# WeltXing/PyDyNet

Measured on AMD Instinct MI355X. Metric: training-step samples/sec (6L Llama3, seq=256), higher is better.
Workload: dtype f32

## Files before the change

### pydynet_amd/csrc/common.h

```cpp
#pragma once
#include <hip/hip_runtime.h>
#include <stdint.h>
#include <stdio.h>
#include <string.h>

#define PDN_MAX_DIMS 8

enum {
  PDN_OK = 0,
  PDN_EINVAL = -1,
  PDN_EUNSUPPORTED = -2,
  PDN_EWORKSPACE = -3,
};

void pdn_set_error(const char* fmt, ...);

enum {
  PDN_CNT_ROWRES_CHUNK = 0,
  PDN_CNT_ROWTILE_PLAIN = 1,
  PDN_CNT_ROWTILE_SWIGLU_FWD = 2,
  PDN_CNT_ROWTILE_SWIGLU_BWD = 3,
  PDN_CNT_ROWTILE_ROPE = 4,
  PDN_CNT_ROWTILE_ROWMAX = 5,
  PDN_CNT_ROWRES_CHUNK_EPI = 6,
  PDN_CNT_ATT_P_FWD = 7,
  PDN_CNT_ATT_P_BWD = 8,
  PDN_CNT_ATT_RES_FWD = 9,
  PDN_CNT_ATT_RES_BWD = 10,
  PDN_CNT_ATT_STREAM = 11,
  PDN_CNT_CE_DX_DEFERRED = 12,
  PDN_CNT_CE_DW = 13,
  PDN_CNT_OUTRES = 14,
  PDN_CNT_OUTRES_TN = 15,
  PDN_CNT_LINEAR_RELU_FWD = 16,
  PDN_CNT_LINEAR_DX_MASKED = 17,
  PDN_CNT_CE_SMALL = 18,
  PDN_CNT_TILED_SWIGLU_FWD = 19,
  PDN_CNT_TILED_SWIGLU_BWD = 20,
  PDN_CNT_CONV_QUAD_FWD = 21,
  PDN_CNT_CONV_QUAD_DGRAD = 22,
  PDN_CNT_CONV_QUAD_WGRAD = 23,
  PDN_CNT_PATCH_EMBED_FWD = 24,
  PDN_CNT_PATCH_EMBED_BWD = 25,
  PDN_CNT_L2NORM_FWD = 26,
  PDN_CNT_L2NORM_BWD = 27,
  PDN_CNT_SAMPLE = 28,
  PDN_CNT_DECODE_ROWS = 29,
  PDN_CNT_DECODE_SLOTS = 30,
  PDN_CNT_DECODE_WIDE = 31,
  PDN_CNT_BEAM = 32,
  PDN_CNT_EXTEND = 33,
  PDN_CNT_SPECULATE = 34,
  PDN_CNT_PENALTY = 35,
  PDN_CNT_LOGPROBS = 36,
  PDN_CNT_LMHEAD_SPLIT = 37,
  PDN_CNT_PREFIX = 38,
  PDN_CNT_CE_DX_SPLIT = 39,
  PDN_CNT_CE_DW_SPLIT = 40,
  PDN_CNT_ROWTILE_SPLIT = 41,
  PDN_CNT_OUTRES_TN_SPLIT = 42,
  PDN_CNT_ATT_SEG = 43,
  PDN_CNT_ROW_LOSS = 44,
  PDN_CNT_SMOOTH_LOSS = 45,
  PDN_CNT_OUTRES_SPLIT = 46,
  PDN_CNT_PROJ288_SPLIT = 47,
  PDN_CNT_LOGIT_EDIT = 48,
  PDN_CNT_PERSAMPLE = 49,
  PDN_CNT_SLOTS = 50
};
void pdn_count(int slot);

#define PDN_CHECK_ARG(cond, ...)          \
  do {                                    \
    if (!(cond)) {                        \
      pdn_set_error(__VA_ARGS__);         \
      return PDN_EINVAL;                  \
    }                                     \
  } while (0)

#define PDN_LAUNCH_CHECK()                                            \
  do {                                                                \
    hipError_t _e = hipGetLastError();                                \
    if (_e != hipSuccess) {                                           \
      pdn_set_error("%s:%d launch failed: %s", __FILE__, __LINE__,    \
                    hipGetErrorString(_e));                           \
      return (int)_e;                                                 \
    }                                                                 \
  } while (0)

#define PDN_HIP(call)                                                 \
  do {                                                                \
    hipError_t _e = (call);                                           \
    if (_e != hipSuccess) {                                           \
      pdn_set_error("%s:%d %s: %s", __FILE__, __LINE__, #call,        \
                    hipGetErrorString(_e));                           \
      return (int)_e;                                                 \
    }                                                                 \
  } while (0)

static inline int64_t cdiv64(int64_t a, int64_t b) { return (a + b - 1) / b; }

struct PdnView {
  int ndim;
  int64_t shape[PDN_MAX_DIMS];
  int64_t stride[PDN_MAX_DIMS];
};

__device__ __forceinline__ float wave_sum(float v) {
#pragma unroll
  for (int o = 32; o > 0; o >>= 1) v += __shfl_xor(v, o, 64);
  return v;
}
__device__ __forceinline__ float wave_max(float v) {
#pragma unroll
  for (int o = 32; o > 0; o >>= 1) v = fmaxf(v, __shfl_xor(v, o, 64));
  return v;
}
__device__ __forceinline__ double wave_sum(double v) {
#pragma unroll
  for (int o = 32; o > 0; o >>= 1) v += __shfl_xor(v, o, 64);
  return v;
}

template <typename T>
__device__ __forceinline__ T block_sum(T v, T* smem) {
  v = wave_sum(v);
  const int lane = threadIdx.x & 63, wid = threadIdx.x >> 6, nw = (blockDim.x + 63) >> 6;
  if (nw == 1) return v;
  __syncthreads();
  if (lane == 0) smem[wid] = v;
  __syncthreads();
  T r = (T)0;
  for (int i = 0; i < nw; ++i) r += smem[i];
  return r;
}
__device__ __forceinline__ void lds_barrier() {
  asm volatile("s_waitcnt lgkmcnt(0)" ::: "memory");
  __builtin_amdgcn_s_barrier();
  asm volatile("" ::: "memory");
}
__device__ __forceinline__ float block_sum_lds(float v, float* smem) {
  v = wave_sum(v);
  const int lane = threadIdx.x & 63, wid = threadIdx.x >> 6, nw = (blockDim.x + 63) >> 6;
  if (nw == 1) return v;
  lds_barrier();
  if (lane == 0) smem[wid] = v;
  lds_barrier();
  float r = 0.f;
  for (int i = 0; i < nw; ++i) r += smem[i];
  return r;
}
// ... 23 lines not shown
```

### pydynet_amd/csrc/gemm.hip

```cpp
#include "common.h"
#include <vector>
#include <mutex>
#include <stdlib.h>
#include <stdio.h>
#include <type_traits>

#include "gemm_tiled.h"
#include "gemm_stream.h"
#include "split_tn.h"

struct TileCfg {
  int waves_m, waves_n, wm, wn, bk;
  float eff;
};
static const TileCfg kCfgs[] = {
    {2, 2, 2, 2, 32, 1.00f},
    {4, 1, 1, 3, 32, 0.97f},
    {1, 4, 3, 1, 32, 0.95f},
    {4, 1, 1, 2, 32, 0.85f},
    {1, 4, 2, 1, 32, 0.90f},
    {2, 2, 1, 1, 32, 0.60f},
    {2, 2, 4, 2, 16, 0.85f},
    {2, 2, 2, 4, 16, 1.10f},
    {4, 1, 2, 3, 16, 0.99f},
// ... 57 lines not shown
    PDN_HIP(hipEventSynchronize(r.e1));
    float t = 0.f;
    PDN_HIP(hipEventElapsedTime(&t, r.e0, r.e1));
    tm += t; tf += r.flops; tb += r.bytes; n++;
    (void)hipEventDestroy(r.e0);
    (void)hipEventDestroy(r.e1);
  }
  g_prof.swap(keep);
  if (ms) *ms = tm;
  if (flops) *flops = tf;
  if (bytes) *bytes = tb;
  if (launches) *launches = n;
  return PDN_OK;
}

#define PDN_GEMM_FAMILIES 5
extern "C" int pdn_gemm_prof_collect_families(double* ms5, double* flops5, int64_t* launches5) {
  std::lock_guard<std::mutex> lk(g_prof_mu);
  double ms[PDN_GEMM_FAMILIES] = {0}, fl[PDN_GEMM_FAMILIES] = {0};
  int64_t n[PDN_GEMM_FAMILIES] = {0};
  for (auto& r : g_prof) {
    PDN_HIP(hipEventSynchronize(r.e1));
    float t = 0.f;
    PDN_HIP(hipEventElapsedTime(&t, r.e0, r.e1));
    const int f = r.family == 5 ? 2 : (r.family < 0 || r.family >= PDN_GEMM_FAMILIES ? 0 : r.family);
    ms[f] += t; fl[f] += r.flops; n[f]++;
    (void)hipEventDestroy(r.e0);
    (void)hipEventDestroy(r.e1);
  }
  for (int f = 0; f < PDN_GEMM_FAMILIES; ++f) {
    if (ms5) ms5[f] = ms[f];
    if (flops5) flops5[f] = fl[f];
    if (launches5) launches5[f] = n[f];
  }
  g_prof.clear();
  return PDN_OK;
}

extern "C" int pdn_gemm_prof_collect(double* total_ms, double* total_flops, int64_t* launches) {
  double ms[PDN_GEMM_FAMILIES], fl[PDN_GEMM_FAMILIES];
  int64_t n[PDN_GEMM_FAMILIES];
  int rc = pdn_gemm_prof_collect_families(ms, fl, n);
  if (rc) return rc;
  double tm = 0, tf = 0;
  int64_t tn = 0;
  for (int f = 0; f < PDN_GEMM_FAMILIES; ++f) { tm += ms[f]; tf += fl[f]; tn += n[f]; }
  if (total_ms) *total_ms = tm;
  if (total_flops) *total_flops = tf;
  if (launches) *launches = tn;
  return PDN_OK;
}

int pdn_gemm_outres_tn_plan(int N, int K, int* nw_out, int* k_per_split_out);
int pdn_gemm_outres_tn_launch(const float* X, const float* G, float* C, int N, int K, int64_t ldx, int64_t ldg,
                              int64_t ldc, int64_t slab, int nw, int k_per_split, void* stream);
int pdn_gemm_outres_tn_blocks_launch(const float* X, const float* G, float* C, int N, int K, int64_t ldx, int64_t ldg,
                                     int nb_cols, int nw, int k_per_split, void* stream);
extern "C" int64_t pdn_gemm_outres_workspace_bytes(int M, int K);
extern "C" int pdn_gemm_outres_plan(int M, int K, int* nw, int* kps);
extern "C" int pdn_gemm_outres_ws_f32(const float* A, const float* B, float* C, const float* bias, const float* residual,
                                      int M, int N, int K, int64_t lda, int64_t ldb, int64_t ldc, int b_trans,
                                      void* workspace, int64_t workspace_bytes, void* stream);
extern "C" int pdn_gemm_outres_supported(int M, int N, int K, int64_t lda, int64_t ldb, int64_t ldc, int b_trans);
extern "C" int pdn_gemm_outres_f32(const float* A, const float* B, float* C, const float* bias,
                                   const float* residual, int M, int N, int K, int64_t lda, int64_t ldb,
                                   int64_t ldc, int b_trans, void* stream);
extern "C" int pdn_gemm_rowres_supported(int M, int N, int K, int64_t lda, int64_t ldb, int64_t ldc, int b_trans);
int pdn_rowtile_plain_ok(int M, int N, int b_trans);
extern "C" int pdn_gemm_rowtile_mode(int mode);
int pdn_outres_split_takes(const float* A, const float* B, const float* C, const float* bias, const float* residual, int M,
                           int K, int64_t lda, int64_t ldb, int64_t ldc, int b_trans, int kb, int64_t b_bstride, int splits,
                           void* stream);
int pdn_outres_split_launch(const float* A, const float* B, float* C, const float* bias, const float* residual, int M, int K,
                            int64_t lda, int64_t ldb, int64_t ldc, int b_trans, int kb, int64_t b_bstride, void* stream,
                            int count_slot);
extern "C" int pdn_gemm_rowres_f32(const float* A, const float* B, float* C, const float* bias,
                                   const float* residual, int M, int N, int K, int64_t lda, int64_t ldb,
                                   int64_t ldc, int b_trans, void* stream);
int pdn_gemm_rowres_blocks(const float* A, const float* B, float* C, int M, int N, int K, int64_t lda, int64_t ldb,
                           int64_t ldc, int b_trans, int nblocks, int64_t b_block_stride, void* stream);

extern "C" int64_t pdn_gemm_f32_workspace_bytes(int M, int N, int K, int nbatch) {
  const int64_t base = (int64_t)64 * M * N * (int64_t)nbatch * 4;
  if (!pdn_outres_tn_split_supported(M, N, nbatch, K)) return base;
  return ((base + 255) & ~(int64_t)255) + pdn_outres_tn_split_extra_bytes(K);
}

bool pdn_gemm_narrow_nn_ok(int M, int N, int K, int64_t a_rs, int64_t a_cs, const void* A);
int pdn_gemm_narrow_nn_launch(const float* A, int64_t lda, const float* B, int64_t b_rs, int64_t b_cs, const float* bias,
                              float* C, int64_t ldc, int M, int N, int K, void* stream);
int pdn_gemm_narrow_tn_plan(int Mc, int N, int K, int64_t a_rs, int64_t a_cs, int64_t b_cs, const void* A, int64_t ws_cap_floats,
                            int* kps);
int pdn_gemm_narrow_tn_launch(const float* A, int64_t a_cs, const float* B, int64_t b_rs, float* slabs, int Mc, int N, int K,
                              int kps, int splits, void* stream);

static int gemm_f32_impl(int M, int N, int K, float alpha, const float* A, int64_t a_rs,
                         int64_t a_cs, const float* B, int64_t b_rs, int64_t b_cs, float beta,
                         float* C, int64_t ldc, const float* bias, int nb1, int nb2,
                         int64_t a_bs1, int64_t a_bs2, int64_t b_bs1, int64_t b_bs2,
                         int64_t c_bs1, int64_t c_bs2, const float* residual,
                         float* b_colsum, int colsum_accumulate, void* workspace,
                         int64_t workspace_bytes, void* stream, uint32_t* relu_mask, const uint32_t* grad_mask,
                         float* mask_colsum = nullptr) {
  const bool ext_on = relu_mask || grad_mask;
  PDN_CHECK_ARG(!ext_on || (nb1 == 1 && nb2 == 1 && N % 32 == 0 && !b_colsum),
                "pdn_gemm_f32: the mask epilogues need one batch and N a multiple of 32 (N = %d)", N);
  PDN_CHECK_ARG(M >= 0 && N >= 0 && K >= 0 && nb1 >= 0 && nb2 >= 0, "pdn_gemm_f32: negative extent");
  if (M == 0 || N == 0 || nb1 == 0 || nb2 == 0) return PDN_OK;
  PDN_CHECK_ARG(A && B && C, "pdn_gemm_f32: null operand");
  PDN_CHECK_ARG(ldc >= N, "pdn_gemm_f32: ldc (%lld) < N (%d)", (long long)ldc, N);
  hipStream_t st = (hipStream_t)stream;
  const int nbatch = nb1 * nb2;

  GemmParams p;
  p.A = A; p.B = B; p.C = C; p.bias = bias; p.ws = (float*)workspace;
  p.residual = residual; p.colsum = b_colsum; p.colsum_acc = colsum_accumulate;
  p.relu_mask = relu_mask; p.grad_mask = grad_mask; p.mask_colsum = grad_mask ? mask_colsum : nullptr;
  p.M = M; p.N = N; p.K = K;
  p.a_rs = a_rs; p.a_cs = a_cs; p.b_rs = b_rs; p.b_cs = b_cs; p.ldc = ldc;
  p.nb2 = nb2;
  p.a_bs1 = a_bs1; p.a_bs2 = a_bs2; p.b_bs1 = b_bs1; p.b_bs2 = b_bs2; p.c_bs1 = c_bs1; p.c_bs2 = c_bs2;
  p.alpha = alpha; p.beta = beta;

  const bool a_kin = !(a_rs == 1 && a_cs != 1) || M == 1;
  const bool b_kin = (b_rs == 1 && b_cs != 1) || (b_rs == 1 && N == 1);
  auto al16 = [](const void* q) { return ((uintptr_t)q & 15) == 0; };
  auto m4 = [](int64_t v) { return (v & 3) == 0; };
  bool vec = al16(A) && al16(B) && m4(a_bs1) && m4(a_bs2) && m4(b_bs1) && m4(b_bs2);
  if (a_kin) vec = vec && a_cs == 1 && m4(a_rs) && m4(K);
  else vec = vec && a_rs == 1 && m4(a_cs) && m4(M);
  if (b_kin) vec = vec && b_rs == 1 && m4(b_cs) && m4(K);
  else vec = vec && b_cs == 1 && m4(b_rs) && m4(N);

  if (b_colsum) {
    if (a_kin || b_kin || !vec || nbatch != 1) {
      pdn_set_error("pdn_gemm_f32: b_colsum needs the x^T @ g layout (A m-contiguous, B n-contiguous, aligned, unbatched)");
      return PDN_EUNSUPPORTED;
    }
  }
  if (M <= 4 && !ext_on && nbatch == 1 && !b_colsum && b_cs == 1 && a_cs == 1 && m4(N) && m4(b_rs) && m4(ldc) &&
      al16(B) && al16(C) && (!bias || al16(bias)) && (!residual || al16(residual)) && K > 0 &&
      (K <= 4096 || (int64_t)K <= 4ll * N)) {
    const dim3 g((N + 127) / 128);
    switch (M) {
      case 1: hipLaunchKernelGGL((gemm_skinny_kernel<1>), g, dim3(256), 0, st, p); break;
      case 2: hipLaunchKernelGGL((gemm_skinny_kernel<2>), g, dim3(256), 0, st, p); break;
      case 3: hipLaunchKernelGGL((gemm_skinny_kernel<3>), g, dim3(256), 0, st, p); break;
      default: hipLaunchKernelGGL((gemm_skinny_kernel<4>), g, dim3(256), 0, st, p); break;
    }
    PDN_LAUNCH_CHECK();
    return PDN_OK;
  }
  if (nbatch == 1 && !ext_on && N <= 16 && alpha == 1.f && !residual && !b_colsum && !getenv("PDN_GEMM_NO_NARROW")) {
    if (beta == 0.f && pdn_gemm_narrow_nn_ok(M, N, K, a_rs, a_cs, A)) {
      if (getenv("PDN_GEMM_DEBUG")) fprintf(stderr, "pdn_gemm_f32 M=%d N=%d K=%d -> narrow NN\n", M, N, K);
      return pdn_gemm_narrow_nn_launch(A, a_rs, B, b_rs, b_cs, bias, C, ldc, M, N, K, stream);
    }
    int kps = 0;
    const int64_t cap = (workspace && workspace_bytes > 0 && al16(workspace)) ? workspace_bytes / 4 : 0;
    const int sp = !bias ? pdn_gemm_narrow_tn_plan(M, N, K, a_rs, a_cs, b_cs, A, cap, &kps) : 0;
    if (sp > 0) {
      if (getenv("PDN_GEMM_DEBUG")) fprintf(stderr, "pdn_gemm_f32 M=%d N=%d K=%d -> narrow TN (%d slabs)\n", M, N, K, sp);
      const int rc = pdn_gemm_narrow_tn_launch(A, a_cs, B, b_rs, (float*)workspace, M, N, K, kps, sp, stream);
      if (rc) return rc;
      p.splits = sp;
      const int64_t total = (int64_t)M * N;
      const int blocks = (int)((total + 255) / 256 < 2048 ? (total + 255) / 256 : 2048);
// ... 115 lines not shown
        std::lock_guard<std::mutex> lk(g_prof_mu);
        prof = g_prof_on;
      }
      if (prof) {
        PDN_HIP(hipEventCreate(&rec.e0));
        PDN_HIP(hipEventCreate(&rec.e1));
        rec.flops = 2.0 * M * (double)N * (double)K;
        rec.family = 4;
        PDN_HIP(hipEventRecord(rec.e0, st));
      }
      if (getenv("PDN_GEMM_DEBUG"))
        fprintf(stderr, "pdn_gemm_f32 M=%d N=%d K=%d -> output-resident TN (splits %d)\n", M, N, K, splits);
      int rc = direct ? pdn_gemm_outres_tn_launch(A, B, C, N, K, a_cs, b_rs, ldc, 0, nw, kps, stream)
                      : pdn_gemm_outres_tn_launch(A, B, (float*)workspace, N, K, a_cs, b_rs, N, (int64_t)M * N, nw, kps, stream);
      if (rc) return rc;
      if (!direct) {
        p.splits = splits;
        const int64_t total = (int64_t)M * N;
        const int blocks = (int)((total + 255) / 256 < 2048 ? (total + 255) / 256 : 2048);
        const int rvec = (ldc % 4 == 0) && al16(C) && al16(workspace);
        hipLaunchKernelGGL(gemm_splitk_reduce_kernel, dim3(blocks), dim3(256), 0, st, p, 1, rvec);
        PDN_LAUNCH_CHECK();
      }
      if (prof) {
        PDN_HIP(hipEventRecord(rec.e1, st));
        std::lock_guard<std::mutex> lk(g_prof_mu);
        g_prof.push_back(rec);
      }
      return PDN_OK;
    }
  }
  {
    const bool one_dim = nb1 == 1 || nb2 == 1;
    const int64_t a_bs = nb1 == 1 ? a_bs2 : a_bs1, b_bs = nb1 == 1 ? b_bs2 : b_bs1;
    const int64_t n_all = (int64_t)N * nbatch;
    if (nbatch > 1 && one_dim && M == 288 && a_bs == 0 && b_bs == N && a_rs == 1 && a_cs >= 288 && b_cs == 1 &&
        b_rs >= n_all && alpha == 1.f && !b_colsum && !bias && !residual && N % 32 == 0 && n_all >= 768 && n_all <= 8192 &&
        K % 32 == 0 && K >= 16384 && m4(a_cs) && m4(b_rs) && al16(A) && al16(B) && !getenv("PDN_GEMM_NO_OUTRES")) {
      int nw = 8, kps = K;
      int splits = pdn_gemm_outres_tn_plan((int)n_all, K, &nw, &kps);
      const int64_t xoff = (((int64_t)64 * M * n_all * 4 + 255) & ~(int64_t)255);
      const bool split16 = pdn_outres_tn_split_supported(M, N, nbatch, K) && pdn_outres_tn_split_enabled() && workspace &&
                           workspace_bytes >= xoff + pdn_outres_tn_split_extra_bytes(K) && al16(workspace);
      if (split16) {
        kps = ((K / 32 + pdn_outres_tn_split_ranges((int)n_all, K, splits) - 1) / pdn_outres_tn_split_ranges((int)n_all, K, splits)) * 32;
        splits = (K + kps - 1) / kps;
      }
      if (splits > 1 && (int64_t)splits * M * n_all <= ws_cap && nbatch * splits <= 65535) {
        bool prof;
        ProfRec rec;
        {
          std::lock_guard<std::mutex> lk(g_prof_mu);
          prof = g_prof_on;
        }
        if (prof) {
          PDN_HIP(hipEventCreate(&rec.e0));
          PDN_HIP(hipEventCreate(&rec.e1));
          rec.flops = 2.0 * M * (double)n_all * (double)K;
          rec.family = 4;
          PDN_HIP(hipEventRecord(rec.e0, st));
        }
        if (getenv("PDN_GEMM_DEBUG"))
          fprintf(stderr, "pdn_gemm_f32 M=%d N=%lld K=%d -> output-resident TN%s (%d blocks, splits %d)\n", M,
                  (long long)n_all, K, split16 ? ", split-fp16" : "", nbatch, splits);
        int rc = split16 ? pdn_outres_tn_split_launch(A, B, (float*)workspace, (int)n_all, K, a_cs, b_rs, N, kps,
                                                      (char*)workspace + xoff, stream)
                         : pdn_gemm_outres_tn_blocks_launch(A, B, (float*)workspace, (int)n_all, K, a_cs, b_rs, N, nw, kps, stream);
        if (rc) return rc;
        p.splits = splits;
        const int64_t total = (int64_t)M * n_all;
        const int blocks = (int)((total + 255) / 256 < 2048 ? (total + 255) / 256 : 2048);
        const int rvec = (ldc % 4 == 0) && al16(C) && m4(c_bs1) && m4(c_bs2) && al16(workspace);
        hipLaunchKernelGGL(gemm_splitk_reduce_kernel, dim3(blocks), dim3(256), 0, st, p, nbatch, rvec);
        PDN_LAUNCH_CHECK();
        if (prof) {
          PDN_HIP(hipEventRecord(rec.e1, st));
          std::lock_guard<std::mutex> lk(g_prof_mu);
          g_prof.push_back(rec);
        }
        return PDN_OK;
      }
    }
  }
  constexpr int SNW = 8;
  bool use_stream = false;
  int sshape = 0;
  bool stream_fits = (int64_t)M * N * nbatch <= (getenv("PDN_GEMM_STREAM_MAX") ? atol(getenv("PDN_GEMM_STREAM_MAX")) : (1 << 20) - 1);
  if (stream_fits && (int64_t)M * N * nbatch >= (1 << 18) && !getenv("PDN_GEMM_STREAM_MAX")) {
    static const int kPadTiles[3][2] = {{128, 128}, {128, 96}, {96, 128}};
    double pad = 1e30;
    for (const auto& t : kPadTiles)
      pad = std::min(pad, (double)(cdiv64(M, t[0]) * t[0]) * (double)(cdiv64(N, t[1]) * t[1]) / ((double)M * N));
    stream_fits = pad > 1.04;
  }
  if (!ext_on && !a_kin && !b_kin && a_rs == 1 && b_cs == 1 && !b_colsum && K >= 2048 && stream_fits && nbatch <= 64 &&
      !getenv("PDN_GEMM_NO_STREAM")) {
    static const int kShapes[5][2] = {{3, 3}, {5, 2}, {2, 5}, {4, 2}, {2, 4}};
    static const double kShapeCost[5] = {1.0, 1.05, 1.08, 1.07, 1.02};
    sshape = 0;
    if (vec) {
      double best_area = (double)cdiv64(M, 96) * cdiv64(N, 96) * 96 * 96 * ((M % 96 == 0 && N % 96 == 0) ? 0.975 : 1.0);
      for (int c = 1; c < 5; ++c) {
        const int th = kShapes[c][0] * 32, tw = kShapes[c][1] * 32;
        const double area = (double)cdiv64(M, th) * cdiv64(N, tw) * th * tw * kShapeCost[c];
        if (area < best_area) { best_area = area; sshape = c; }
      }
      if (const char* e = getenv("PDN_GEMM_STREAM_SHAPE")) { const int c = atoi(e); if (c >= 0 && c < 5) sshape = c; }
    }
    const int sth = kShapes[sshape][0] * 32, stw = kShapes[sshape][1] * 32;
    const int tm = (int)cdiv64(M, sth), tn = (int)cdiv64(N, stw), tiles = tm * tn * nbatch;
    if (tiles <= 256) {
      double best_cost = 1e300;
      int best_kps = 0, best_sp = 1;
      const int smax = (int)std::min<int64_t>(64, K / (SNW * 16));
      for (int s = 1; s <= smax; ++s) {
        if (s > 1 && (int64_t)s * M * N * nbatch > ws_cap) break;
        const int kw = (int)cdiv64(cdiv64(K, (int64_t)s * SNW), 8) * 8;
        const int kps = kw * SNW, sp = (int)cdiv64(K, kps);
        const double rounds = (double)cdiv64((int64_t)tiles * sp, 256);
        double cost = rounds * (kw * 0.5 * (kShapes[sshape][0] * kShapes[sshape][1]) * 64 * (SNW / 4.0) + 6000.0);
        if (sp > 1) cost += (double)sp * M * N * nbatch * 8.0 / 1700.0 + 5000.0;
        if (cost < best_cost) { best_cost = cost; best_kps = kps; best_sp = sp; }
      }
      if (const char* e = getenv("PDN_GEMM_STREAM_SPLITS")) {
        const int s = atoi(e);
        if (s >= 1 && (s == 1 || (int64_t)s * M * N * nbatch <= ws_cap)) {
          const int kw = (int)cdiv64(cdiv64(K, (int64_t)s * SNW), 8) * 8;
          best_kps = kw * SNW; best_sp = (int)cdiv64(K, best_kps);
        }
      }
      use_stream = true;
      p.tiles_m = tm; p.tiles_n = tn; p.k_per_split = best_kps; p.splits = best_sp;
    }
  }

  int best = -1, best_splits = 1;
  double best_cost = 1e300;
  static const bool no_fixed = getenv("PDN_GEMM_NO_FIXED") != nullptr;
  for (int c = 0; c < kNumCfgs && !use_stream; ++c) {
    if (!vec && c != kScalarCfg) continue;
    if (ext_on && !(c == 0 || c == 3 || c == 6 || c == 7 || c == 8 || c == kScalarCfg)) continue;
    if (mask_colsum && c == 8) continue;
    if (c == 7 && N < 2048 && !(ext_on && N >= 1024 && N % 256 == 0 && M >= 16384)) continue;
    if (c == 6 && ext_on && !(N >= 1024 && M >= 16384)) continue;
    if (c == 8 && N < 768) continue;
    const int BM = kCfgs[c].waves_m * kCfgs[c].wm * 32, BN = kCfgs[c].waves_n * kCfgs[c].wn * 32;
    const int bk = kCfgs[c].bk;
    const int64_t tiles = cdiv64(M, BM) * cdiv64(N, BN) * nbatch;
    if (c == 12 && !(tiles > 512 && tiles <= 768 && K <= 1024 && a_kin && !b_kin)) continue;
    const int ktiles = (int)cdiv64(K > 0 ? K : 1, bk);
    for (int s = 1; s <= 64; s *= 2) {
      if (s > 1 && (b_colsum || ext_on)) break;
      if (s > 1) {
        if (ktiles * bk / s < 128) break;
        if ((int64_t)s * M * N * nbatch > ws_cap) break;
      }
      const int kps = (int)cdiv64(ktiles, s);
      const double waves_pb = kCfgs[c].waves_m * kCfgs[c].waves_n;
      const double blocks = (double)tiles * s;
      const double slots = 256.0 * (4.0 / waves_pb);
      const double rounds = blocks >= 4 * slots ? blocks / slots : (double)cdiv64((int64_t)blocks, (int64_t)slots);
      const double wps = blocks * waves_pb / 1024.0;
      const double util = wps >= 1.875 ? 1.0 : (wps > 1.0 ? 0.7 + 0.3 * (wps - 1.0) / 0.875 : 0.7);
      const double eff = kCfgs[c].eff;
      double cost = rounds * ((double)BM * BN * (kps * bk + 64) / waves_pb * 4.0 / (eff * util));
      if (!no_fixed) {
// ... 403 lines not shown
```

### pydynet_amd/csrc/outres_tn_split.hip

```cpp
#include "split_tn.h"

struct OtsParams {
  const float* g;
  const char* ximg;
  const int* xsh;
  float* C;
  int n_all, nb_cols, K, k_per_split;
  int64_t ldg, slab, blk_stride;
};

__device__ __forceinline__ unsigned ots_finite_bits(float v) {
  const unsigned b = __float_as_uint(v) & 0x7fffffffu;
  return b < 0x7f800000u ? b : 0u;
}
__device__ __forceinline__ unsigned ots_wave_max_bits(const float (&v)[8]) {
  unsigned m = ots_finite_bits(v[0]);
#pragma unroll
  for (int k = 1; k < 8; ++k) m = max(m, ots_finite_bits(v[k]));
  m = max(m, (unsigned)__builtin_amdgcn_update_dpp(0, (int)m, 0xB1, 0xf, 0xf, false));
  m = max(m, (unsigned)__builtin_amdgcn_update_dpp(0, (int)m, 0x4E, 0xf, 0xf, false));
  m = max(m, (unsigned)__builtin_amdgcn_update_dpp(0, (int)m, 0x141, 0xf, 0xf, false));
  m = max(m, (unsigned)__builtin_amdgcn_update_dpp(0, (int)m, 0x140, 0xf, 0xf, false));
  const unsigned a = __builtin_amdgcn_readlane((int)m, 0), b = __builtin_amdgcn_readlane((int)m, 16);
  const unsigned c = __builtin_amdgcn_readlane((int)m, 32), d = __builtin_amdgcn_readlane((int)m, 48);
  return max(max(a, b), max(c, d));
}

__device__ __forceinline__ void ots_form2(float g0, float g1, int S, unsigned& hp, unsigned& lp) {
  f16x2 h, l;
  _Float16 a, b;
  ls_split_scaled(ldexpf(g0, S), a, b);
  h[0] = a; l[0] = b;
  ls_split_scaled(ldexpf(g1, S), a, b);
  h[1] = a; l[1] = b;
  hp = __builtin_bit_cast(unsigned, h);
  lp = __builtin_bit_cast(unsigned, l);
  asm volatile("" : "+v"(hp), "+v"(lp));
}

template <int ABLATE>
__global__ __launch_bounds__(512, 1) void ots_main_kernel(OtsParams p) {
  __shared__ __attribute__((aligned(1024))) char smem[stn_lds(OTS_XKIB)];
  const int tid = threadIdx.x, lane = tid & 63;
  const int wave = __builtin_amdgcn_readfirstlane(tid >> 6);
  const int r = lane & 15, q = lane >> 4;
  const int bx = blockIdx.x, by = blockIdx.y;
  const int k_begin = by * p.k_per_split;
  const int np = stn_range_pieces(p.K, p.k_per_split, by);
  const int c0 = bx * STN_COLS + wave * 16;
  const bool active = c0 < p.n_all;
  const int col = c0 + r;
  const unsigned lds0 = (unsigned)(size_t)(__attribute__((address_space(3))) char*)smem;

  const char* xsrc = p.ximg + (int64_t)(k_begin / STN_KP) * stn_xpiece(OTS_XKIB);
  auto dma_x = [&](int piece, int slot) __attribute__((always_inline)) {
#pragma unroll
    for (int e = 0; e < 5; ++e) {
      const int I = stn_x_dma_kib(e, wave, OTS_XKIB);
      split_dma16(xsrc + stn_x_dma_src(piece, I, lane, OTS_XKIB), __builtin_amdgcn_readfirstlane(lds0 + stn_x_dma_lds(slot, I, 0, OTS_XKIB)));
    }
  };
  const float* gsrc[2];
#pragma unroll
  for (int i = 0; i < 2; ++i) {
    const int I = stn_raw_dma_kib(i, wave);
    gsrc[i] = p.g + stn_raw_src(k_begin, 0, 1, stn_raw_dma_row(I, lane), p.ldg, stn_raw_col(bx, stn_raw_dma_chunk(I, lane), p.n_all));
  }
  auto dma_g = [&](int piece, int ring) __attribute__((always_inline)) {
    const int64_t o = (int64_t)min(piece, np - 1) * STN_KP * p.ldg;
#pragma unroll
    for (int i = 0; i < 2; ++i)
      split_dma16(gsrc[i] + o, __builtin_amdgcn_readfirstlane(lds0 + stn_raw_dma_lds(ring, stn_raw_dma_kib(i, wave), 0, OTS_XKIB)));
  };
  const int g_lane = stn_raw_read(0, wave, r, q, 0, OTS_XKIB);

  dma_x(0, 0);
  if (ABLATE != 1) { dma_g(0, 0); dma_g(1, 1); dma_g(2, 2); dma_g(3, 3); }
  asm volatile("s_waitcnt vmcnt(0)" ::: "memory");
  __builtin_amdgcn_s_barrier();
  asm volatile("" ::: "memory");
  f16x8 bh, bl;
#pragma unroll
  for (int j = 0; j < 8; ++j) { bh[j] = (_Float16)1.f; bl[j] = (_Float16)0.5f; }
  int S = OTS_S_UNSET;
  if (ABLATE != 1) {
    float rv[8];
#pragma unroll
    for (int k = 0; k < 8; ++k) rv[k] = *reinterpret_cast<const float*>(smem + g_lane + k * 512);
    S = ots_next_scale(ots_wave_max_bits(rv), S);
    unsigned hh[4], ll[4];
#pragma unroll
    for (int e = 0; e < 4; ++e) ots_form2(rv[2 * e], rv[2 * e + 1], S, hh[e], ll[e]);
    bh = stn_pack4(hh[0], hh[1], hh[2], hh[3]); bl = stn_pack4(ll[0], ll[1], ll[2], ll[3]);
  }

  f32x4 acc0[STN_NT], acc1[STN_NT];
  STN_CLEAR(acc0, acc1)

  const int frag = stn_x_frag(0, r, q);
  constexpr int TOPWAIT = ABLATE == 0 ? 2 : 0;

  int cur = 0;
  for (int s = 0; s < np; ++s) {
    asm volatile("s_waitcnt vmcnt(%0)" ::"n"(TOPWAIT) : "memory");
    __builtin_amdgcn_s_barrier();
    asm volatile("" ::: "memory");
    const char* fb = smem + cur + frag;
    const char* raw = smem + g_lane + ((s + 1) & (STN_RING - 1)) * STN_RAW;
    f16x8 xh[2], xl[2];
    u32x4 nh = __builtin_bit_cast(u32x4, bh), nl = __builtin_bit_cast(u32x4, bl);
    float rv[8] = {0.f, 0.f, 0.f, 0.f, 0.f, 0.f, 0.f, 0.f};
    int Sn = S;
    stn_load_frag(fb, 0, xh[0], xl[0]);
#pragma unroll
    for (int j = 0; j < STN_NT; ++j) {
      if (j + 1 < STN_NT) stn_load_frag(fb, j + 1, xh[(j + 1) & 1], xl[(j + 1) & 1]);
      if (j == 0) {
        dma_x(min(s + 1, np - 1), 1 - (cur != 0));
        if (ABLATE == 0) dma_g(s + 4, s & (STN_RING - 1));
        if (ABLATE != 1) {
#pragma unroll
          for (int k = 0; k < 8; ++k) rv[k] = *reinterpret_cast<const float*>(raw + k * 512);
        }
      }
      if (ABLATE != 1 && j == 2) Sn = ots_next_scale(ots_wave_max_bits(rv), S);
      __builtin_amdgcn_sched_barrier(0);
      stn_mfma3(xh[j & 1], xl[j & 1], bh, bl, acc0[j], acc1[j]);
      if (ABLATE != 1 && (j & 3) == 0 && j >= 4) {
        const int e = (j >> 2) - 1;
        unsigned hp, lp;
        ots_form2(rv[2 * e], rv[2 * e + 1], Sn, hp, lp);
        if (e == 0) { nh.x = hp; nl.x = lp; } else if (e == 1) { nh.y = hp; nl.y = lp; }
        else if (e == 2) { nh.z = hp; nl.z = lp; } else { nh.w = hp; nl.w = lp; }
        stn_sched_pair();
      }
      __builtin_amdgcn_sched_barrier(0);
    }
    bh = __builtin_bit_cast(f16x8, nh); bl = __builtin_bit_cast(f16x8, nl);
    if (Sn != S) {
      if (S != OTS_S_UNSET) {
        const int dS = Sn - S;
#pragma unroll
        for (int j = 0; j < STN_NT; ++j)
#pragma unroll
          for (int i = 0; i < 4; ++i) { acc0[j][i] = ldexpf(acc0[j][i], dS); acc1[j][i] = ldexpf(acc1[j][i], dS); }
      }
      S = Sn;
    }
    cur = cur ? 0 : stn_xpiece(OTS_XKIB);
  }
  asm volatile("s_waitcnt vmcnt(0)" ::: "memory");

  if (!active) return;
  const int Se = S == OTS_S_UNSET ? 0 : S;
  const int* __restrict__ shp = p.xsh + 4 * q;
#pragma unroll
  for (int j = 0; j < STN_NT; ++j) {
    const int4 sv = *reinterpret_cast<const int4*>(shp + 16 * j);
    const int sh[4] = {sv.x, sv.y, sv.z, sv.w};
#pragma unroll
    for (int i = 0; i < 4; ++i)
      p.C[ots_out_elem(by, p.slab, p.blk_stride, p.nb_cols, stn_out_row(j, q, i), col)] =
          stn_unscale(acc1[j][i], acc0[j][i], Se + sh[i]);
  }
}

int pdn_outres_tn_split_enabled() {
  static const int s_on = ls_env_switch("PDN_OUTRES_TN_SPLIT", 1, "the packed layer weight gradients stay on the fp32 MFMA kernel");
  return s_on;
}
int pdn_outres_tn_split_supported(int M, int nb_cols, int nbatch, int K) {
  const int64_t n_all = (int64_t)nb_cols * nbatch;
  return (M == STN_N && nbatch > 1 && nb_cols % 16 == 0 && n_all >= 768 && n_all <= 8192 && K >= OTS_MIN_K && K % STN_KP == 0) ? 1 : 0;
}
int64_t pdn_outres_tn_split_extra_bytes(int K) { return stn_extra_bytes(K, OTS_XKIB); }
int pdn_outres_tn_split_ranges(int n_all, int K, int plan) { return ots_ranges(n_all, plan, K / STN_KP); }

int pdn_outres_tn_split_launch(const float* X, const float* G, float* C, int n_all, int K, int64_t ldx, int64_t ldg,
                               int nb_cols, int k_per_split, void* extra, void* stream) {
  PDN_CHECK_ARG(n_all % nb_cols == 0 && pdn_outres_tn_split_supported(STN_N, nb_cols, n_all / nb_cols, K) && k_per_split > 0 &&
                    k_per_split % STN_KP == 0 && ((((uintptr_t)X | (uintptr_t)G | (uintptr_t)extra | (uintptr_t)C) & 15) == 0) &&
                    (ldx & 3) == 0 && (ldg & 3) == 0 && ldx >= STN_N && ldg >= n_all,
                "pdn_outres_tn_split_launch: unsupported shape or alignment (K %d, columns %d)", K, n_all);
  static const int s_ablate = ls_env_switch("PDN_OUTRES_TN_SPLIT_ABLATE", 0,
                                            "timing ablation active, the split packed layer weight gradients are WRONG");
  const int ranges = (K + k_per_split - 1) / k_per_split;
  PDN_CHECK_ARG(ranges <= 65535, "pdn_outres_tn_split_launch: %d K ranges", ranges);
  OtsParams p;
  memset(&p, 0, sizeof(p));
  p.g = G; p.ximg = static_cast<const char*>(extra); p.xsh = stn_x_planes_launch(X, ldx, K, extra, nullptr, nullptr, stream);
  p.C = C;
  p.n_all = n_all; p.nb_cols = nb_cols; p.K = K; p.k_per_split = k_per_split;
  p.ldg = ldg; p.slab = (int64_t)STN_N * nb_cols; p.blk_stride = (int64_t)ranges * STN_N * nb_cols;
  STN_LAUNCH_ABLATE(ots_main_kernel, s_ablate, dim3((unsigned)((n_all + STN_COLS - 1) / STN_COLS), (unsigned)ranges), stream, p);
  pdn_count(PDN_CNT_OUTRES_TN);
  pdn_count(PDN_CNT_OUTRES_TN_SPLIT);
  PDN_LAUNCH_CHECK();
  return PDN_OK;
}
```

### pydynet_amd/csrc/split_tn.h

```cpp
#pragma once
#include "common.h"
#include "lm_head_split.h"
#include "split_tn_index.h"

int* stn_x_planes_launch(const float* x, int64_t ldx, int rows, void* extra, const float* lse, const int64_t* targets, void* stream);
int pdn_outres_tn_split_enabled();
int pdn_outres_tn_split_supported(int M, int nb_cols, int nbatch, int K);
int64_t pdn_outres_tn_split_extra_bytes(int K);
int pdn_outres_tn_split_ranges(int n_all, int K, int plan);
int pdn_outres_tn_split_launch(const float* X, const float* G, float* C, int n_all, int K, int64_t ldx, int64_t ldg,
                               int nb_cols, int k_per_split, void* extra, void* stream);
int pdn_outres_ce_dw_split_enabled();
int pdn_outres_ce_dw_split_supported(int64_t rows, int V, int in_features);
int64_t pdn_outres_ce_dw_split_extra_bytes(int64_t rows);
int pdn_outres_ce_dw_split_launch(const float* x, int64_t ldx, const float* logits, float* C, int V, int64_t rows,
                                  int64_t slab, int k_per_split, const float* lse, const int64_t* targets, float gscale,
                                  const float* gdev, float* colsum, void* extra, void* stream);

typedef float f32x4 __attribute__((ext_vector_type(4)));
typedef _Float16 f16x8 __attribute__((ext_vector_type(8)));
typedef _Float16 f16x2 __attribute__((ext_vector_type(2)));
typedef unsigned u32x4 __attribute__((ext_vector_type(4)));

__device__ __forceinline__ void split_dma16(const void* g, unsigned lds) {
  asm volatile("s_mov_b32 m0, %1\n\ts_nop 0\n\tglobal_load_lds_dwordx4 %0, off" ::"v"(g), "s"(lds) : "memory");
}

__device__ __forceinline__ void stn_load_frag(const char* fb, int J, f16x8& h, f16x8& l) {
  h = *reinterpret_cast<const f16x8*>(__builtin_assume_aligned(fb + J * 1024, 16));
  l = *reinterpret_cast<const f16x8*>(__builtin_assume_aligned(fb + J * 1024 + STN_PLANE, 16));
}
__device__ __forceinline__ void stn_mfma3(f16x8 xh, f16x8 xl, f16x8 bh, f16x8 bl, f32x4& acc0, f32x4& acc1) {
  acc0 = __builtin_amdgcn_mfma_f32_16x16x32_f16(xh, bh, acc0, 0, 0, 0);
  acc1 = __builtin_amdgcn_mfma_f32_16x16x32_f16(xl, bh, acc1, 0, 0, 0);
  acc1 = __builtin_amdgcn_mfma_f32_16x16x32_f16(xh, bl, acc1, 0, 0, 0);
}
__device__ __forceinline__ void stn_sched_pair() {
  __builtin_amdgcn_sched_group_barrier(0x008, 1, 0);
  __builtin_amdgcn_sched_group_barrier(0x002, 8, 0);
  __builtin_amdgcn_sched_group_barrier(0x008, 1, 0);
  __builtin_amdgcn_sched_group_barrier(0x002, 8, 0);
  __builtin_amdgcn_sched_group_barrier(0x008, 1, 0);
}
__device__ __forceinline__ f16x8 stn_pack4(unsigned w0, unsigned w1, unsigned w2, unsigned w3) {
  const u32x4 v = {w0, w1, w2, w3};
  return __builtin_bit_cast(f16x8, v);
}
#define STN_CLEAR(acc0, acc1)                                                \
  _Pragma("unroll") for (int j_ = 0; j_ < STN_NT; ++j_)                      \
    _Pragma("unroll") for (int i_ = 0; i_ < 4; ++i_) { acc0[j_][i_] = 0.f; acc1[j_][i_] = 0.f; }
__device__ __forceinline__ float stn_unscale(float a1, float a0, int e) { return ldexpf(fmaf(a1, 1.f / 2048.f, a0), -e); }

#define STN_LAUNCH_ABLATE(K, ablate, grid, stream, p)                                              \
  do {                                                                                             \
    if ((ablate) == 1) hipLaunchKernelGGL(K<1>, grid, dim3(512), 0, (hipStream_t)(stream), p);     \
    else if ((ablate) == 2) hipLaunchKernelGGL(K<2>, grid, dim3(512), 0, (hipStream_t)(stream), p); \
    else hipLaunchKernelGGL(K<0>, grid, dim3(512), 0, (hipStream_t)(stream), p);                   \
  } while (0)
```

### pydynet_amd/csrc/split_tn_index.h

```cpp
#pragma once
#include <stdint.h>

#if defined(__HIPCC__) || defined(__CUDACC__)
#define STN_HD __host__ __device__ __forceinline__ constexpr
#else
#define STN_HD inline constexpr
#endif

#define STN_N 288
#define STN_NT 18
#define STN_KP 32
#define STN_PLANE (STN_N * STN_KP * 2)
#define STN_COLS 128
#define STN_RAW (STN_KP * STN_COLS * 4)
#define STN_RAWDMA 16
#define STN_RING 4
#define STN_MAX_PARTIAL 2048

#define LDW_XKIB 37
#define LDW_TAIL (2 * STN_PLANE)
#define LDW_MIN_ROWS 32768
#define LDW_MIN_V 128

#define OTS_XKIB 36
#define OTS_MIN_K 32768
#define OTS_MAX_RANGES 64
#define OTS_S_UNSET (1 << 20)
#define OTS_S_TOP 15
#define OTS_S_AIM 12

STN_HD int stn_min_i(int a, int b) { return a < b ? a : b; }

STN_HD int stn_xpiece(int xkib) { return xkib * 1024; }
STN_HD int stn_ring_base(int xkib) { return 2 * stn_xpiece(xkib); }
STN_HD int stn_lds(int xkib) { return stn_ring_base(xkib) + STN_RING * STN_RAW; }
STN_HD int64_t stn_extra_bytes(int64_t rows, int xkib) { return (rows / STN_KP) * (int64_t)stn_xpiece(xkib) + STN_N * 4; }
STN_HD int stn_partials(int64_t rows) { return stn_min_i(STN_MAX_PARTIAL, (int)(rows / STN_KP)); }
static_assert(stn_xpiece(LDW_XKIB) == 37888 && stn_xpiece(OTS_XKIB) == 36864 && STN_N * 4 == 1152, "bytes per piece, exponents");
static_assert(stn_xpiece(OTS_XKIB) == 2 * STN_PLANE && LDW_TAIL + 1024 == stn_xpiece(LDW_XKIB), "an image is two planes, and a tail");
static_assert(stn_lds(LDW_XKIB) == 141312 && stn_lds(OTS_XKIB) == 139264, "LDS allocations");

STN_HD int stn_x_unit(int d, int q) { return (d * 4 + (q ^ ((d >> 2) & 3))) * 16; }
STN_HD int stn_x_frag(int j, int r, int q) { return j * 1024 + (r * 4 + (q ^ ((r >> 2) & 3))) * 16; }
STN_HD int stn_x_dma_kib(int e, int wave, int xkib) { return stn_min_i(e * 8 + wave, xkib - 1); }
STN_HD int64_t stn_x_dma_src(int64_t piece, int I, int lane, int xkib) { return piece * stn_xpiece(xkib) + I * 1024 + lane * 16; }
STN_HD int stn_x_dma_lds(int slot, int I, int lane, int xkib) { return slot * stn_xpiece(xkib) + I * 1024 + lane * 16; }
STN_HD int ldw_tail_nl(int slot, int t) { return slot * stn_xpiece(LDW_XKIB) + LDW_TAIL + 4 * t; }
STN_HD int ldw_tail_tg(int slot, int t) { return slot * stn_xpiece(LDW_XKIB) + LDW_TAIL + 128 + 4 * t; }

STN_HD int stn_raw_dma_kib(int i, int wave) { return wave + 8 * i; }
STN_HD int stn_raw_dma_row(int I, int lane) { return 2 * I + (lane >> 5); }
STN_HD int stn_raw_swz(int t) { return 4 * (t >> 3); }
STN_HD int stn_raw_dma_chunk(int I, int lane) { return (lane & 31) ^ stn_raw_swz(stn_raw_dma_row(I, lane)); }
STN_HD int stn_raw_dma_lds(int ring, int I, int lane, int xkib) { return stn_ring_base(xkib) + ring * STN_RAW + I * 1024 + lane * 16; }
STN_HD int stn_raw_col(int bx, int c, int ncols) { return stn_min_i(bx * STN_COLS + 4 * c, ncols - 4); }
STN_HD int64_t stn_raw_row(int k_begin, int piece, int np, int t) { return (int64_t)k_begin + (int64_t)stn_min_i(piece, np - 1) * STN_KP + t; }
STN_HD int64_t stn_raw_src(int k_begin, int piece, int np, int t, int64_t ld, int col) { return stn_raw_row(k_begin, piece, np, t) * ld + col; }
STN_HD int stn_raw_read(int ring, int wave, int r, int q, int k, int xkib) {
  const int t = 8 * q + k;
  return stn_ring_base(xkib) + ring * STN_RAW + t * 512 + (((4 * wave + (r >> 2)) ^ stn_raw_swz(t)) << 4) + 4 * (r & 3);
}

STN_HD int ots_next_scale(unsigned mbits, int S) {
  if (mbits == 0u) return S;
  const int E = (int)(mbits >> 23);
  return (E - 127 + S >= OTS_S_TOP) ? (OTS_S_AIM + 127 - E) : S;
}

STN_HD int stn_range_pieces(int K, int k_per_split, int by) {
  const int b = by * k_per_split, e = stn_min_i(K, b + k_per_split);
  return (e - b) / STN_KP;
}
STN_HD int ots_ranges(int n_all, int plan, int pieces) {
  const int cb = (n_all + STN_COLS - 1) / STN_COLS;
  const int lo = stn_min_i(plan, OTS_MAX_RANGES);
  const int rounds = (cb * lo + 255) / 256;
  int r = stn_min_i(OTS_MAX_RANGES, rounds * 256 / cb);
  if (r < lo) r = lo;
  if (r > pieces) r = pieces;
  return r < 1 ? 1 : r;
}
STN_HD int ots_k_per_split(int pieces, int ranges) { return ((pieces + ranges - 1) / ranges) * STN_KP; }
STN_HD int stn_out_row(int j, int q, int i) { return 16 * j + 4 * q + i; }
STN_HD int64_t ldw_out_elem(int by, int64_t slab, int d, int V, int col) { return (int64_t)by * slab + (int64_t)d * V + col; }
STN_HD int64_t ots_out_elem(int by, int64_t slab, int64_t blk_stride, int nb_cols, int d, int col) {
  const int b = col / nb_cols;
  return (int64_t)b * blk_stride + (int64_t)by * slab + (int64_t)d * nb_cols + (col - b * nb_cols);
}
```

### pydynet_amd/csrc/split_tn_planes.hip

```cpp
#include "split_tn.h"

#define STN_L2E 1.4426950408889634f

__global__ __launch_bounds__(288) void stn_x_colmax_kernel(const float* __restrict__ x, int64_t ldx, int rows, int rows_per_block,
                                                            float* __restrict__ partial) {
  __shared__ float sm[4][STN_N];
  const int c4 = threadIdx.x % 72, g = threadIdx.x / 72;
  const int r0 = blockIdx.x * rows_per_block, r1 = min(rows, r0 + rows_per_block);
  float4 m = make_float4(0.f, 0.f, 0.f, 0.f);
  float4 z = m;
#pragma unroll 4
  for (int r = r0 + g; r < r1; r += 4) {
    const float4 v = *reinterpret_cast<const float4*>(x + (int64_t)r * ldx + 4 * c4);
    m.x = fmaxf(m.x, fabsf(v.x)); m.y = fmaxf(m.y, fabsf(v.y)); m.z = fmaxf(m.z, fabsf(v.z)); m.w = fmaxf(m.w, fabsf(v.w));
    z.x = fmaf(v.x, 0.f, z.x); z.y = fmaf(v.y, 0.f, z.y); z.z = fmaf(v.z, 0.f, z.z); z.w = fmaf(v.w, 0.f, z.w);
  }
  if (z.x != z.x) m.x = INFINITY;
  if (z.y != z.y) m.y = INFINITY;
  if (z.z != z.z) m.z = INFINITY;
  if (z.w != z.w) m.w = INFINITY;
  sm[g][4 * c4 + 0] = m.x; sm[g][4 * c4 + 1] = m.y; sm[g][4 * c4 + 2] = m.z; sm[g][4 * c4 + 3] = m.w;
  __syncthreads();
  const int d = threadIdx.x;
  partial[(int64_t)blockIdx.x * STN_N + d] = fmaxf(fmaxf(sm[0][d], sm[1][d]), fmaxf(sm[2][d], sm[3][d]));
}

__global__ __launch_bounds__(256) void stn_x_shift_kernel(const float* __restrict__ partial, int nparts, int* __restrict__ xsh) {
  __shared__ float sm[4];
  const int d = blockIdx.x;
  float m = 0.f;
  for (int b = threadIdx.x; b < nparts; b += 256) m = fmaxf(m, partial[(int64_t)b * STN_N + d]);
  m = wave_max(m);
  if ((threadIdx.x & 63) == 0) sm[threadIdx.x >> 6] = m;
  __syncthreads();
  if (threadIdx.x == 0) xsh[d] = ls_shift(fmaxf(fmaxf(sm[0], sm[1]), fmaxf(sm[2], sm[3])));
}

template <int XKIB, bool TAIL>
__device__ __forceinline__ void stn_split_x(const float* __restrict__ x, int64_t ldx, const int* __restrict__ xsh,
                                            const float* __restrict__ lse, const int64_t* __restrict__ targets, int rows,
                                            char* __restrict__ ximg) {
  char* img = ximg + (int64_t)blockIdx.x * stn_xpiece(XKIB);
  const float* xp = x + (int64_t)blockIdx.x * STN_KP * ldx;
  for (int i = threadIdx.x; i < STN_N * 4; i += 256) {
    const int d = i % STN_N, q = i / STN_N;
    const int sh = xsh[d];
    f16x8 hv, lv;
#pragma unroll
    for (int k = 0; k < 8; ++k) {
      _Float16 h, l;
      ls_split(xp[(int64_t)(8 * q + k) * ldx + d], sh, h, l);
      hv[k] = h; lv[k] = l;
    }
    char* dst = img + stn_x_unit(d, q);
    *reinterpret_cast<f16x8*>(dst) = hv;
    *reinterpret_cast<f16x8*>(dst + STN_PLANE) = lv;
  }
  if (TAIL) {
    const int i = threadIdx.x;
    const int64_t t = ((int64_t)blockIdx.x + 1) * STN_KP + (i & 31);
    unsigned v = 0u;
    if (i < 64 && t < rows) v = i < 32 ? __float_as_uint(-STN_L2E * lse[t]) : (unsigned)(int)targets[t];
    reinterpret_cast<unsigned*>(img + LDW_TAIL)[i] = v;
  }
}
__global__ __launch_bounds__(256) void stn_split_x_kernel(const float* __restrict__ x, int64_t ldx, const int* __restrict__ xsh,
                                                           char* __restrict__ ximg) {
  stn_split_x<OTS_XKIB, false>(x, ldx, xsh, nullptr, nullptr, 0, ximg);
}
__global__ __launch_bounds__(256) void stn_split_x_tail_kernel(const float* __restrict__ x, int64_t ldx, const int* __restrict__ xsh,
                                                                const float* __restrict__ lse, const int64_t* __restrict__ targets,
                                                                int rows, char* __restrict__ ximg) {
  stn_split_x<LDW_XKIB, true>(x, ldx, xsh, lse, targets, rows, ximg);
}

int* stn_x_planes_launch(const float* x, int64_t ldx, int rows, void* extra, const float* lse, const int64_t* targets, void* stream) {
  hipStream_t st = (hipStream_t)stream;
  const bool tail = lse != nullptr;
  const int npieces = rows / STN_KP;
  char* ximg = static_cast<char*>(extra);
  int* xsh = reinterpret_cast<int*>(ximg + (int64_t)npieces * stn_xpiece(tail ? LDW_XKIB : OTS_XKIB));
  float* partial = reinterpret_cast<float*>(ximg);
  const int nparts = stn_partials(rows);
  const int rpb = (rows + nparts - 1) / nparts;
  const int nblk = (rows + rpb - 1) / rpb;
  hipLaunchKernelGGL(stn_x_colmax_kernel, dim3(nblk), dim3(288), 0, st, x, ldx, rows, rpb, partial);
  hipLaunchKernelGGL(stn_x_shift_kernel, dim3(STN_N), dim3(256), 0, st, partial, nblk, xsh);
  if (tail) hipLaunchKernelGGL(stn_split_x_tail_kernel, dim3(npieces), dim3(256), 0, st, x, ldx, xsh, lse, targets, rows, ximg);
  else hipLaunchKernelGGL(stn_split_x_kernel, dim3(npieces), dim3(256), 0, st, x, ldx, xsh, ximg);
  return xsh;
}
```

Measured before the change: 8721.

## Route down-projection weight-grad GEMM through split-fp16 output-resident TN kernel

Adds a transposed variant of the output-resident TN split kernel that handles the down-projection weight gradient (N equal to the model width, M 512–1024). It splits the fp32 operand into fp16 hi/lo planes for matrix-core use, computes K-range partials, and reduces them with the existing split-K reduce. Partial outputs are written with a transposed float4 store. The x-plane split kernel now stages rows through LDS with coalesced float4 loads before converting, instead of strided scalar global reads. The cost is extra workspace, several extra launches (colmax, shift, split, reduce) and reliance on hi/lo fp16 accuracy.

```diff
diff --git a/pydynet_amd/csrc/common.h b/pydynet_amd/csrc/common.h
--- a/pydynet_amd/csrc/common.h
+++ b/pydynet_amd/csrc/common.h
@@ -66,7 +66,8 @@
   PDN_CNT_PROJ288_SPLIT = 47,
   PDN_CNT_LOGIT_EDIT = 48,
   PDN_CNT_PERSAMPLE = 49,
-  PDN_CNT_SLOTS = 50
+  PDN_CNT_DOWN_DW_SPLIT = 50,
+  PDN_CNT_SLOTS = 51
 };
 void pdn_count(int slot);
 
diff --git a/pydynet_amd/csrc/gemm.hip b/pydynet_amd/csrc/gemm.hip
--- a/pydynet_amd/csrc/gemm.hip
+++ b/pydynet_amd/csrc/gemm.hip
@@ -163,7 +163,7 @@
 
 extern "C" int64_t pdn_gemm_f32_workspace_bytes(int M, int N, int K, int nbatch) {
   const int64_t base = (int64_t)64 * M * N * (int64_t)nbatch * 4;
-  if (!pdn_outres_tn_split_supported(M, N, nbatch, K)) return base;
+  if (!pdn_outres_tn_split_supported(M, N, nbatch, K) && !(nbatch == 1 && pdn_down_dw_split_supported(M, N, K))) return base;
   return ((base + 255) & ~(int64_t)255) + pdn_outres_tn_split_extra_bytes(K);
 }
 
@@ -445,6 +445,29 @@
       }
     }
   }
+  if (nbatch == 1 && !ext_on && a_rs == 1 && b_cs == 1 && alpha == 1.f && !b_colsum && !bias && !residual &&
+      pdn_down_dw_split_supported(M, N, K) && a_cs >= M && b_rs >= N && m4(a_cs) && m4(b_rs) && al16(A) && al16(B) && workspace &&
+      al16(workspace) && pdn_outres_tn_split_enabled() && !getenv("PDN_GEMM_NO_OUTRES")) {
+    const int64_t xoff = (((int64_t)64 * M * N * 4 + 255) & ~(int64_t)255);
+    const int ranges = pdn_down_dw_split_ranges(M, K);
+    const int kps = ((K / 32 + ranges - 1) / ranges) * 32;
+    const int splits = (K + kps - 1) / kps;
+    if (workspace_bytes >= xoff + pdn_outres_tn_split_extra_bytes(K) && splits > 1 && splits <= 64) {
+      if (getenv("PDN_GEMM_DEBUG"))
+        fprintf(stderr, "pdn_gemm_f32 M=%d N=%d K=%d -> output-resident TN, split-fp16, transposed (splits %d)\n", M, N, K, splits);
+      const int tk = pdn_gemm_prof_begin(4, 2.0 * M * (double)N * (double)K, 0.0, stream);
+      const int rc = pdn_down_dw_split_launch(B, A, (float*)workspace, M, K, b_rs, a_cs, kps, (char*)workspace + xoff, stream);
+      if (rc) { pdn_gemm_prof_end(tk, stream); return rc; }
+      p.splits = splits;
+      const int64_t total = (int64_t)M * N;
+      const int blocks = (int)((total + 255) / 256 < 2048 ? (total + 255) / 256 : 2048);
+      const int rvec = (ldc % 4 == 0) && al16(C);
+      hipLaunchKernelGGL(gemm_splitk_reduce_kernel, dim3(blocks), dim3(256), 0, st, p, 1, rvec);
+      PDN_LAUNCH_CHECK();
+      pdn_gemm_prof_end(tk, stream);
+      return PDN_OK;
+    }
+  }
   constexpr int SNW = 8;
   bool use_stream = false;
   int sshape = 0;
diff --git a/pydynet_amd/csrc/outres_tn_split.hip b/pydynet_amd/csrc/outres_tn_split.hip
--- a/pydynet_amd/csrc/outres_tn_split.hip
+++ b/pydynet_amd/csrc/outres_tn_split.hip
@@ -38,7 +38,7 @@
   asm volatile("" : "+v"(hp), "+v"(lp));
 }
 
-template <int ABLATE>
+template <int ABLATE, bool TSTORE = false>
 __global__ __launch_bounds__(512, 1) void ots_main_kernel(OtsParams p) {
   __shared__ __attribute__((aligned(1024))) char smem[stn_lds(OTS_XKIB)];
   const int tid = threadIdx.x, lane = tid & 63;
@@ -158,10 +158,17 @@
   for (int j = 0; j < STN_NT; ++j) {
     const int4 sv = *reinterpret_cast<const int4*>(shp + 16 * j);
     const int sh[4] = {sv.x, sv.y, sv.z, sv.w};
-#pragma unroll
-    for (int i = 0; i < 4; ++i)
-      p.C[ots_out_elem(by, p.slab, p.blk_stride, p.nb_cols, stn_out_row(j, q, i), col)] =
-          stn_unscale(acc1[j][i], acc0[j][i], Se + sh[i]);
+    if (TSTORE) {
+      float4 o;
+      o.x = stn_unscale(acc1[j][0], acc0[j][0], Se + sh[0]); o.y = stn_unscale(acc1[j][1], acc0[j][1], Se + sh[1]);
+      o.z = stn_unscale(acc1[j][2], acc0[j][2], Se + sh[2]); o.w = stn_unscale(acc1[j][3], acc0[j][3], Se + sh[3]);
+      *reinterpret_cast<float4*>(p.C + ots_out_elem_t(by, p.slab, stn_out_row(j, q, 0), col)) = o;
+    } else {
+#pragma unroll
+      for (int i = 0; i < 4; ++i)
+        p.C[ots_out_elem(by, p.slab, p.blk_stride, p.nb_cols, stn_out_row(j, q, i), col)] =
+            stn_unscale(acc1[j][i], acc0[j][i], Se + sh[i]);
+    }
   }
 }
 
@@ -198,3 +205,29 @@
   PDN_LAUNCH_CHECK();
   return PDN_OK;
 }
+
+int pdn_down_dw_split_supported(int M, int N, int K) {
+  return (N == STN_N && M % 16 == 0 && M >= 512 && M <= 1024 && K >= OTS_MIN_K && K % STN_KP == 0) ? 1 : 0;
+}
+int pdn_down_dw_split_ranges(int M, int K) { return ots_t_ranges(M, K / STN_KP); }
+
+int pdn_down_dw_split_launch(const float* G2, const float* H, float* C, int M, int K, int64_t ldx, int64_t ldg, int k_per_split,
+                             void* extra, void* stream) {
+  PDN_CHECK_ARG(pdn_down_dw_split_supported(M, STN_N, K) && k_per_split > 0 && k_per_split % STN_KP == 0 &&
+                    ((((uintptr_t)G2 | (uintptr_t)H | (uintptr_t)extra | (uintptr_t)C) & 15) == 0) && (ldx & 3) == 0 &&
+                    (ldg & 3) == 0 && ldx >= STN_N && ldg >= M,
+                "pdn_down_dw_split_launch: unsupported shape or alignment (K %d, rows %d)", K, M);
+  const int ranges = (K + k_per_split - 1) / k_per_split;
+  PDN_CHECK_ARG(ranges <= OTS_MAX_RANGES, "pdn_down_dw_split_launch: %d K ranges", ranges);
+  OtsParams p;
+  memset(&p, 0, sizeof(p));
+  p.g = H; p.ximg = static_cast<const char*>(extra); p.xsh = stn_x_planes_launch(G2, ldx, K, extra, nullptr, nullptr, stream);
+  p.C = C;
+  p.n_all = M; p.nb_cols = M; p.K = K; p.k_per_split = k_per_split;
+  p.ldg = ldg; p.slab = (int64_t)STN_N * M; p.blk_stride = 0;
+  hipLaunchKernelGGL((ots_main_kernel<0, true>), dim3((unsigned)((M + STN_COLS - 1) / STN_COLS), (unsigned)ranges), dim3(512), 0,
+                     (hipStream_t)stream, p);
+  pdn_count(PDN_CNT_DOWN_DW_SPLIT);
+  PDN_LAUNCH_CHECK();
+  return PDN_OK;
+}
diff --git a/pydynet_amd/csrc/split_tn.h b/pydynet_amd/csrc/split_tn.h
--- a/pydynet_amd/csrc/split_tn.h
+++ b/pydynet_amd/csrc/split_tn.h
@@ -10,6 +10,10 @@
 int pdn_outres_tn_split_ranges(int n_all, int K, int plan);
 int pdn_outres_tn_split_launch(const float* X, const float* G, float* C, int n_all, int K, int64_t ldx, int64_t ldg,
                                int nb_cols, int k_per_split, void* extra, void* stream);
+int pdn_down_dw_split_supported(int M, int N, int K);
+int pdn_down_dw_split_ranges(int M, int K);
+int pdn_down_dw_split_launch(const float* G2, const float* H, float* C, int M, int K, int64_t ldx, int64_t ldg, int k_per_split,
+                             void* extra, void* stream);
 int pdn_outres_ce_dw_split_enabled();
 int pdn_outres_ce_dw_split_supported(int64_t rows, int V, int in_features);
 int64_t pdn_outres_ce_dw_split_extra_bytes(int64_t rows);
diff --git a/pydynet_amd/csrc/split_tn_index.h b/pydynet_amd/csrc/split_tn_index.h
--- a/pydynet_amd/csrc/split_tn_index.h
+++ b/pydynet_amd/csrc/split_tn_index.h
@@ -45,6 +45,18 @@
 STN_HD int stn_x_dma_kib(int e, int wave, int xkib) { return stn_min_i(e * 8 + wave, xkib - 1); }
 STN_HD int64_t stn_x_dma_src(int64_t piece, int I, int lane, int xkib) { return piece * stn_xpiece(xkib) + I * 1024 + lane * 16; }
 STN_HD int stn_x_dma_lds(int slot, int I, int lane, int xkib) { return slot * stn_xpiece(xkib) + I * 1024 + lane * 16; }
+#define STN_PASS_THREADS 256
+#define STN_PASS_LOADS (STN_KP * STN_N / 4 / STN_PASS_THREADS)
+STN_HD int stn_pass_row(int i) { return i / (STN_N / 4); }
+STN_HD int stn_pass_chunk(int i) { return i % (STN_N / 4); }
+STN_HD int stn_pass_lds(int t, int d) {
+  const int c = (d >> 2) + 4 * (t >> 3);
+  return t * STN_N + 4 * (c >= STN_N / 4 ? c - STN_N / 4 : c) + (d & 3);
+}
+STN_HD int stn_pass_unit_d(int u) { return u >> 2; }
+STN_HD int stn_pass_unit_q(int u) { return (u & 3) ^ ((u >> 4) & 3); }
+static_assert(STN_PASS_LOADS * STN_PASS_THREADS * 4 == STN_KP * STN_N, "nine whole load items per thread");
+
 STN_HD int ldw_tail_nl(int slot, int t) { return slot * stn_xpiece(LDW_XKIB) + LDW_TAIL + 4 * t; }
 STN_HD int ldw_tail_tg(int slot, int t) { return slot * stn_xpiece(LDW_XKIB) + LDW_TAIL + 128 + 4 * t; }
 
@@ -81,6 +93,13 @@
   return r < 1 ? 1 : r;
 }
 STN_HD int ots_k_per_split(int pieces, int ranges) { return ((pieces + ranges - 1) / ranges) * STN_KP; }
+STN_HD int ots_t_ranges(int n_all, int pieces) {
+  const int cb = (n_all + STN_COLS - 1) / STN_COLS;
+  int r = stn_min_i(OTS_MAX_RANGES, 256 / cb);
+  if (r > pieces) r = pieces;
+  return r < 1 ? 1 : r;
+}
+STN_HD int64_t ots_out_elem_t(int by, int64_t slab, int d, int col) { return (int64_t)by * slab + (int64_t)col * STN_N + d; }
 STN_HD int stn_out_row(int j, int q, int i) { return 16 * j + 4 * q + i; }
 STN_HD int64_t ldw_out_elem(int by, int64_t slab, int d, int V, int col) { return (int64_t)by * slab + (int64_t)d * V + col; }
 STN_HD int64_t ots_out_elem(int by, int64_t slab, int64_t blk_stride, int nb_cols, int d, int col) {
diff --git a/pydynet_amd/csrc/split_tn_planes.hip b/pydynet_amd/csrc/split_tn_planes.hip
--- a/pydynet_amd/csrc/split_tn_planes.hip
+++ b/pydynet_amd/csrc/split_tn_planes.hip
@@ -40,21 +40,37 @@
 __device__ __forceinline__ void stn_split_x(const float* __restrict__ x, int64_t ldx, const int* __restrict__ xsh,
                                             const float* __restrict__ lse, const int64_t* __restrict__ targets, int rows,
                                             char* __restrict__ ximg) {
+  __shared__ __attribute__((aligned(16))) float raw[STN_KP * STN_N];
   char* img = ximg + (int64_t)blockIdx.x * stn_xpiece(XKIB);
   const float* xp = x + (int64_t)blockIdx.x * STN_KP * ldx;
-  for (int i = threadIdx.x; i < STN_N * 4; i += 256) {
-    const int d = i % STN_N, q = i / STN_N;
-    const int sh = xsh[d];
-    f16x8 hv, lv;
+  float4 v[STN_PASS_LOADS];
 #pragma unroll
-    for (int k = 0; k < 8; ++k) {
-      _Float16 h, l;
-      ls_split(xp[(int64_t)(8 * q + k) * ldx + d], sh, h, l);
-      hv[k] = h; lv[k] = l;
+  for (int e = 0; e < STN_PASS_LOADS; ++e) {
+    const int i = threadIdx.x + STN_PASS_THREADS * e;
+    v[e] = *reinterpret_cast<const float4*>(xp + (int64_t)stn_pass_row(i) * ldx + 4 * stn_pass_chunk(i));
+  }
+#pragma unroll
+  for (int e = 0; e < STN_PASS_LOADS; ++e) {
+    const int i = threadIdx.x + STN_PASS_THREADS * e;
+    *reinterpret_cast<float4*>(raw + stn_pass_lds(stn_pass_row(i), 4 * stn_pass_chunk(i))) = v[e];
+  }
+  __syncthreads();
+#pragma unroll
+  for (int e = 0; e < (STN_N * 4 + STN_PASS_THREADS - 1) / STN_PASS_THREADS; ++e) {
+    const int u = threadIdx.x + STN_PASS_THREADS * e;
+    if (u < STN_N * 4) {
+      const int d = stn_pass_unit_d(u), q = stn_pass_unit_q(u);
+      const int sh = xsh[d];
+      f16x8 hv, lv;
+#pragma unroll
+      for (int k = 0; k < 8; ++k) {
+        _Float16 h, l;
+        ls_split(raw[stn_pass_lds(8 * q + k, d)], sh, h, l);
+        hv[k] = h; lv[k] = l;
+      }
+      *reinterpret_cast<f16x8*>(img + 16 * u) = hv;
+      *reinterpret_cast<f16x8*>(img + STN_PLANE + 16 * u) = lv;
     }
-    char* dst = img + stn_x_unit(d, q);
-    *reinterpret_cast<f16x8*>(dst) = hv;
-    *reinterpret_cast<f16x8*>(dst + STN_PLANE) = lv;
   }
   if (TAIL) {
     const int i = threadIdx.x;
```

After: 9116 (median of 6 runs). 4.5% higher.
